# dfm/emcee

Measured on AMD Instinct MI355X. Metric: walker-updates/sec (whole node), 64-dim correlated Gaussian, StretchMove a=2, higher is better.
Workload: dtype f64

## Files before the change

emcee_amd/csrc/emx_kernels.hpp:

```cpp
#pragma once
#include <hip/hip_runtime.h>

#include <cstdint>
#include <type_traits>

#include "emx_planlog.hpp"
#include "emx_rng.hpp"

#ifndef EMX_OPT_RED4
#define EMX_OPT_RED4 1
#endif
#ifndef EMX_OPT_RTILE
#define EMX_OPT_RTILE 1
#endif
#ifndef EMX_LEAN_FOLD_D
#define EMX_LEAN_FOLD_D 0
#endif
#ifndef EMX_LEAN_FOLD_SPW
#define EMX_LEAN_FOLD_SPW 1
#endif
#ifndef EMX_OPT_SKEW
#define EMX_OPT_SKEW 1
#endif
#ifndef EMX_SNOOKER_BUDGET
#define EMX_SNOOKER_BUDGET 48
#endif
#ifndef EMX_STAMP_WAVE
#define EMX_STAMP_WAVE 0
#endif
#ifndef EMX_OPT_STAMPS
#define EMX_OPT_STAMPS 0
#endif
#ifndef EMX_EXPERIMENTS
#define EMX_EXPERIMENTS 0
#endif

namespace emx {

enum : int { MOVE_STRETCH = 0, MOVE_DE = 1, MOVE_SNOOKER = 2, MOVE_GAUSS = 3, MOVE_EVAL = 4,
             MOVE_WALK = 5, MOVE_KDE = 6,
             MOVE_MIX = 8  };
enum : int { GAUSS_VECTOR = 0, GAUSS_RANDOM = 1, GAUSS_SEQUENTIAL = 2 };
enum : int { TGT_NONE = 0, TGT_ISO = 1, TGT_DIAG = 2, TGT_DENSE = 3, TGT_ROSEN = 4, TGT_BOX = 5,
             TGT_REPLAY = 7, TGT_USER = 8 };
enum : uint32_t { ST_NAN_LOGP = 1u, ST_BAD_COORD = 2u, ST_EXCHANGE_OVERFLOW = 4u, ST_EXCHANGE_TIMEOUT = 8u,
                  ST_PLAN_PRODUCER = 16u,
                  ST_SINGULAR_COV = 32u };
constexpr int EMX_MAX_PEERS = 8;

__device__ __forceinline__ void raise_status(uint32_t* flags, uint32_t bit) {
    __hip_atomic_store(&flags[__builtin_ctz(bit)], 1u, __ATOMIC_RELAXED, __HIP_MEMORY_SCOPE_SYSTEM);
}

struct NativeArgs {
    uint64_t seed;
    uint64_t step;
    PermKey pk;
};

struct StepDesc {
    NativeArgs nat;
    long long stored_idx;
};
struct GraphCounters {
    unsigned long long step_base;
    long long stored_base;
};

struct HalfStepArgs {
    double* X;
    double* lp;
    uint8_t* acc;
    uint32_t* acc_count;
    double* chain;
    double* chain_lp;
    uint32_t* status;
    double* qout;
    double* fout;
    double* sendbuf;
    const int32_t* order;
    const int32_t* p0;
    const int32_t* p1;
    const int32_t* p2;
    const double* s0;
    const double* uacc;
    const double* logu;
    const double* fac;
    const double* tp0;
    const double* tp1;
    double tscale;
    double a;
    double sigma, g0;
    double gammas;
    int32_t N, D, S, split;
    int32_t pos0, ns;
    int32_t t_lo, t_hi;
    int32_t spw;
    int32_t target;
    int32_t Dp;
    int32_t ablate;
    const StepDesc* desc;
    double* chain_all;
    double* chain_lp_all;
    const int32_t* t_hi_dev;
    const double* disp;
    const double* gscale;
    double gsigma, gfac;
    unsigned long long gseed, gstep;
    unsigned long long* dbg;
    const struct PeerTable* peers;
    int32_t npeer;
    double* declp;
    const struct PeerTable* push_peers;
    long long push_off;
    int32_t npush;
    int32_t skew_sleep;
};

struct PeerTable {
    const double* X[EMX_MAX_PEERS];
    int32_t lo[EMX_MAX_PEERS];
};

template <int LEAN>
__device__ __forceinline__ const double* partner_base(const HalfStepArgs& A, int j) {
    if (LEAN == 1 || LEAN == 3 || LEAN == 4 || A.npeer == 0) return A.X;
    const PeerTable* __restrict__ T = A.peers;
    const double* b = T->X[0];
#pragma unroll
    for (int q = 1; q < EMX_MAX_PEERS; ++q) b = (q < A.npeer && j >= T->lo[q]) ? T->X[q] : b;
    return b;
}

template <int CTRL>
__device__ __forceinline__ double dpp_f64(double x) {
    const int lo = __builtin_amdgcn_update_dpp(0, __double2loint(x), CTRL, 0xf, 0xf, false);
    const int hi = __builtin_amdgcn_update_dpp(0, __double2hiint(x), CTRL, 0xf, 0xf, false);
    return __hiloint2double(hi, lo);
}

__device__ __forceinline__ double sum_swap16(double x) {
    const unsigned lo = (unsigned)__double2loint(x), hi = (unsigned)__double2hiint(x);
    const auto a = __builtin_amdgcn_permlane16_swap(lo, lo, false, false);
    const auto b = __builtin_amdgcn_permlane16_swap(hi, hi, false, false);
    return __hiloint2double((int)b[0], (int)a[0]) + __hiloint2double((int)b[1], (int)a[1]);
}

__device__ __forceinline__ double sum_swap32(double x) {
    const unsigned lo = (unsigned)__double2loint(x), hi = (unsigned)__double2hiint(x);
    const auto a = __builtin_amdgcn_permlane32_swap(lo, lo, false, false);
    const auto b = __builtin_amdgcn_permlane32_swap(hi, hi, false, false);
    return __hiloint2double((int)b[0], (int)a[0]) + __hiloint2double((int)b[1], (int)a[1]);
}

template <int G>
__device__ __forceinline__ double group_sum(double x) {
    if constexpr (G >= 2) x += dpp_f64<0xB1>(x);
    if constexpr (G >= 4) x += dpp_f64<0x4E>(x);
    if constexpr (G >= 8) x += dpp_f64<0x141>(x);
    if constexpr (G >= 16) x += dpp_f64<0x140>(x);
    if constexpr (G >= 32) x = sum_swap16(x);
    if constexpr (G >= 64) x = sum_swap32(x);
    return x;
}

__device__ __forceinline__ double row16_sum4(double v0, double v1, double v2, double v3, int lane) {
    const bool b0 = lane & 1, b1 = lane & 2;
    const double x = (b0 ? v1 : v0) + dpp_f64<0xB1>(b0 ? v0 : v1);
    const double y = (b0 ? v3 : v2) + dpp_f64<0xB1>(b0 ? v2 : v3);
    double z = (b1 ? y : x) + dpp_f64<0x4E>(b1 ? x : y);
    z += dpp_f64<0x124>(z);
    z += dpp_f64<0x128>(z);
    return z;
}

template <int G>
__device__ __forceinline__ bool group_any(bool pred, int sub) {
    const unsigned long long m = __ballot(pred);
    if constexpr (G == 64) {
        return m != 0ull;
    } else {
        return ((m >> (sub * G)) & ((1ull << G) - 1ull)) != 0ull;
    }
}
// ... 709 lines not shown
                    EMX_WAVE_SYNC();
                    double my_qf = 0.0;
                    {
                        const int am = lane & 15, ak = lane >> 4;
                        typedef double d4 __attribute__((ext_vector_type(4)));
                        double afr[KK];
#pragma unroll
                        for (int kk = 0; kk < KK; ++kk) {
                            if constexpr (RTILE)
                                afr[kk] = tile[am * RT + 4 * kk + ak];
                            else
                                afr[kk] = tile[am * RT + 4 * kk + ak] - muS[4 * kk + ak];
                        }
                        double part[4] = {0.0, 0.0, 0.0, 0.0};
                        if (EMX_OPT_STAMPS && A.dbg) { asm volatile("s_waitcnt lgkmcnt(0)" ::: "memory"); }
                        EMX_STAMP(5);
                        if (!(ablate_ & 1))
#pragma unroll
                        for (int nb = 0; nb < DPB; ++nb) {
                            d4 accv = {0.0, 0.0, 0.0, 0.0};
#pragma unroll
                            for (int kk = 4 * nb; kk < KK; ++kk)
                                accv = __builtin_amdgcn_mfma_f64_16x16x4f64(afr[kk], Sfrag[(dense_block(DPB, nb, kk >> 2) * 4 + (kk & 3)) * 64 + lane], accv, 0, 0, 0);
#pragma unroll
                            for (int r = 0; r < 4; ++r) part[r] = fma(accv[r], accv[r], part[r]);
                        }
                        if (EMX_OPT_STAMPS && A.dbg) { asm volatile("s_nop 0" ::: "memory"); }
                        EMX_STAMP(6);
#if EMX_OPT_RED4
                        my_qf = row16_sum4(part[0], part[1], part[2], part[3], lane);
#else
#pragma unroll
                        for (int r = 0; r < 4; ++r) part[r] = group_sum<16>(part[r]);
                        my_qf = part[0];
#pragma unroll
                        for (int r = 1; r < 4; ++r) my_qf = (am == r) ? part[r] : my_qf;
#endif
                    }
                    EMX_STAMP(7);
                    bool acc = false;
                    double lp_fin = my_lpo;
                    if (mine) {
                        const double lpn = -0.5 * my_qf;
                        if (lpn != lpn) raise_status(A.status, ST_NAN_LOGP);
                        if constexpr (MOVE == MOVE_EVAL) {
                            A.lp[my_i] = lpn;
                        } else {
                            const double lnpdiff = facS[myrow] + lpn - my_lpo;
                            acc = lnpdiff > my_logu;
                            A.acc[my_i] = acc ? 1 : 0;
                            if (acc) {
                                A.lp[my_i] = lpn;
                                lp_fin = lpn;
                            }
                            if (chain_lp_) {
                                chain_lp_[my_i] = lp_fin;
                                if (acc) A.acc_count[my_i] += 1u;
                            }
                            if (declp_) put_decision(t0 + tb + myrow - tlo_, acc ? lpn : __builtin_nan(""));
                        }
                    }
                    EMX_STAMP(8);
                    if constexpr (MOVE != MOVE_EVAL) {
                        const unsigned long long am64 = __ballot(acc);
                        if (sendbuf_ && (lane & 15) < 4) qfS[myrow] = lp_fin;
                        if (sendbuf_) EMX_WAVE_SYNC();
#pragma unroll
                        for (int pp = 0; pp < PPT; ++pp) {
                            if (ablate_ & 8) break;
                            const int row = pp * WPW + sub;
                            const int sidx = tb + row;
                            const bool lv = sidx < nslot;
                            const bool ac = lv && ((am64 >> ((row & 3) * 16 + (row >> 2))) & 1ull);
                            if (!lv) continue;
                            if (sendbuf_ && gl == 0) {
                                double* sb = sendbuf_ + (size_t)(t0 + sidx - tlo_) * (D + 2);
                                sb[D] = qfS[row];
                                sb[D + 1] = ac ? 1.0 : 0.0;
                            }
                            if (!ac) continue;
                            int wi2;
                            if constexpr (PF == PPT) {
                                wi2 = wi[0];
#pragma unroll
                                for (int k2 = 1; k2 < PF; ++k2) wi2 = (pp == k2) ? wi[k2] : wi2;
                            } else {
                                wi2 = A.order[pbase + sidx];
                            }
                            Row<G, V, CH> rr;
                            if constexpr (RTILE) {
                                rr = qk[pp < PF ? pp : 0];
                            } else {
#pragma unroll
                                for (int c = 0; c < CH; ++c)
#pragma unroll
                                    for (int v = 0; v < V; ++v) {
                                        const int d = (c * G + gl) * V + v;
                                        rr.x[c][v] = d < D ? tile[row * RT + d] : 0.0;
                                    }
                            }
                            store_row<G, V, CH>(rr, A.X + (size_t)wi2 * D, D, gl);
                            if (chain_) store_row_stream<G, V, CH>(rr, chain_ + (size_t)wi2 * D, D, gl);
                            if (sendbuf_) store_row<G, V, CH>(rr, sendbuf_ + (size_t)(t0 + sidx - tlo_) * (D + 2), D, gl);
                        }
                    }
                    EMX_STAMP(9);
                    EMX_WAVE_SYNC();
                }
            }
        }
    }
    if (EMX_OPT_STAMPS && A.dbg) { asm volatile("s_waitcnt vmcnt(0)" ::: "memory"); }
    EMX_STAMP(10);
    if (EMX_OPT_STAMPS && A.dbg && wib == 0 && lane == 0) A.dbg[(size_t)blockIdx.x * 16 + 12] = wall_clock64();
}

typedef unsigned int emx_u4 __attribute__((ext_vector_type(4)));
constexpr int EMX_CPOL_SC1 = 16;
template <int G, int V, int CH, int CPOL = EMX_CPOL_SC1>
__device__ __forceinline__ void load_row_agent(Row<G, V, CH>& r, __amdgpu_buffer_rsrc_t rsrc, int row, int D, int gl) {
    static_assert(V == 2 || V == 1, "two coordinates per lane and chunk (even ndim), or one (odd ndim: rows are 8-byte aligned only)");
    const int base = row * D;
    if constexpr (V == 1) {
        typedef unsigned int emx_u2 __attribute__((ext_vector_type(2)));
#pragma unroll
        for (int c = 0; c < CH; ++c) {
            const int d = c * G + gl;
            if (d < D) {
                const emx_u2 w = __builtin_amdgcn_raw_buffer_load_b64(rsrc, (base + d) * 8, 0, CPOL);
                double t;
                __builtin_memcpy(&t, &w, 8);
                r.x[c][0] = t;
            } else {
                r.x[c][0] = 0.0;
            }
        }
        return;
    }
#pragma unroll
    for (int c = 0; c < CH; ++c) {
        const int d = (c * G + gl) * V;
        if (d + 1 < D) {
            const emx_u4 w = __builtin_amdgcn_raw_buffer_load_b128(rsrc, (base + d) * 8, 0, CPOL);
            double2 t;
            __builtin_memcpy(&t, &w, 16);
            r.x[c][0] = t.x;
            r.x[c][1] = t.y;
        } else {
            r.x[c][0] = 0.0;
            r.x[c][1] = 0.0;
        }
    }
}
template <int G, int V, int CH, int CPOL = EMX_CPOL_SC1>
__device__ __forceinline__ void store_row_agent(const Row<G, V, CH>& r, __amdgpu_buffer_rsrc_t rsrc, int row, int D, int gl) {
    static_assert(V == 2 || V == 1, "two coordinates per lane and chunk (even ndim), or one (odd ndim)");
    const int base = row * D;
    if constexpr (V == 1) {
        typedef unsigned int emx_u2 __attribute__((ext_vector_type(2)));
#pragma unroll
        for (int c = 0; c < CH; ++c) {
            const int d = c * G + gl;
            if (d < D) {
                emx_u2 w;
                const double t = r.x[c][0];
                __builtin_memcpy(&w, &t, 8);
                __builtin_amdgcn_raw_buffer_store_b64(w, rsrc, (base + d) * 8, 0, CPOL);
            }
        }
        return;
    }
#pragma unroll
    for (int c = 0; c < CH; ++c) {
        const int d = (c * G + gl) * V;
        if (d + 1 < D) {
            const double2 t = {r.x[c][0], r.x[c][1]};
            emx_u4 w;
            __builtin_memcpy(&w, &t, 16);
            __builtin_amdgcn_raw_buffer_store_b128(w, rsrc, (base + d) * 8, 0, CPOL);
        }
    }
}
template <typename T>
__device__ __forceinline__ void store_agent(T* p, T v) { __hip_atomic_store(p, v, __ATOMIC_RELAXED, __HIP_MEMORY_SCOPE_AGENT); }
__device__ __forceinline__ double load_agent(const double* p) { return __hip_atomic_load(p, __ATOMIC_RELAXED, __HIP_MEMORY_SCOPE_AGENT); }
__device__ __forceinline__ unsigned load_agent(const unsigned* p) { return __hip_atomic_load(p, __ATOMIC_RELAXED, __HIP_MEMORY_SCOPE_AGENT); }
template <bool LOCAL, typename T>
__device__ __forceinline__ void store_scope(T* p, T v) {
    if constexpr (LOCAL)
        *p = v;
    else
        store_agent(p, v);
}

constexpr int PERSIST_MAX_ITERS = 40;
constexpr int PERSIST_BAR_STRIDE = 32;
constexpr int PERSIST_BAR_WORDS = 12 * PERSIST_BAR_STRIDE;
struct PersistIter {
    const char* plan;
    double *chain, *chain_lp;
    int32_t pos0, split;
    double gammas;
    int32_t kind, shift;
};
struct PersistCols {
    const int32_t *order, *p0, *p1, *p2;
    const double *s0, *logu, *fac;
    double *chain, *chain_lp;
    int32_t pos0, split;
    double gammas;
    int32_t kind, shift;
    __host__ __device__ __forceinline__ PersistCols(const PersistIter& it, size_t N)
        : order(reinterpret_cast<const int32_t*>(it.plan)), p0(reinterpret_cast<const int32_t*>(it.plan) + N),
          p1(reinterpret_cast<const int32_t*>(it.plan + N * 24)), p2(reinterpret_cast<const int32_t*>(it.plan + N * 24) + N),
          s0(reinterpret_cast<const double*>(it.plan + N * 8)), logu(reinterpret_cast<const double*>(it.plan + N * 32)),
          fac(reinterpret_cast<const double*>(it.plan + N * 32) + N), chain(it.chain), chain_lp(it.chain_lp), pos0(it.pos0), split(it.split),
          gammas(it.gammas), kind(it.kind), shift(it.shift) {}
};
struct PersistArgs {
    HalfStepArgs base;
    PersistIter it[PERSIST_MAX_ITERS];
    unsigned* bar;
    unsigned* ver;
    unsigned epoch0;
    unsigned lepoch0;
    unsigned hepoch0;
    unsigned long long timeout_ticks;
    int32_t niter;
    unsigned seq;
    unsigned* started_host;
    int32_t stagger;
};
static_assert(sizeof(PersistArgs) <= 4096, "kernel arguments of the persistent kernels");

__device__ __forceinline__ void persist_barrier_local(const PersistArgs& P, unsigned k, unsigned bid, unsigned ngroups) {
    asm volatile("s_waitcnt vmcnt(0)" ::: "memory");
    __syncthreads();
    if (threadIdx.x < 64) {
        const int lane = threadIdx.x;
        const __amdgpu_buffer_rsrc_t Fr = __builtin_amdgcn_make_buffer_rsrc((void*)(P.bar + 10 * PERSIST_BAR_STRIDE), 0, 64 * 4, 0x00020000);
        if (lane == 0) __builtin_amdgcn_raw_buffer_store_b32(k, Fr, (int)bid * 4, 0, 0);
        const unsigned long long t0 = wall_clock64();
        for (;;) {
            const unsigned v = __builtin_amdgcn_raw_buffer_load_b32(Fr, lane * 4, 0, EMX_CPOL_SC1);
            const bool ok = lane < (int)ngroups ? (int)(v - k) >= 0 : true;
            const bool dead = lane == 32 && v != 0u;
            if (__ballot(ok) == ~0ull || __ballot(dead) != 0ull) break;
            if (wall_clock64() - t0 > P.timeout_ticks) {
                if (lane == 0) {
                    raise_status(P.base.status, ST_EXCHANGE_TIMEOUT);
                    __hip_atomic_store(P.bar + 9 * PERSIST_BAR_STRIDE + 1, 2u, __ATOMIC_RELAXED, __HIP_MEMORY_SCOPE_AGENT);
                    __builtin_amdgcn_raw_buffer_store_b32(1u, Fr, 32 * 4, 0, 0);
                }
                break;
            }
        }
    }
    __syncthreads();
}

__device__ __forceinline__ void persist_barrier(const PersistArgs& P, unsigned k, unsigned long long* wall = nullptr) {
    asm volatile("s_waitcnt vmcnt(0)" ::: "memory");
    __syncthreads();
    if (threadIdx.x == 0) {
        const int xcd = blockIdx.x & 7;
        const unsigned per = (gridDim.x + 7 - xcd) / 8;
        unsigned* xctr = P.bar + xcd * PERSIST_BAR_STRIDE;
        unsigned* gctr = P.bar + 8 * PERSIST_BAR_STRIDE;
        unsigned* go = P.bar + 9 * PERSIST_BAR_STRIDE;
        if (wall) wall[0] = wall_clock64();
        const unsigned old = __hip_atomic_fetch_add(xctr, 1u, __ATOMIC_RELAXED, __HIP_MEMORY_SCOPE_AGENT);
        if (old == k * per - 1) {
            const unsigned o2 = __hip_atomic_fetch_add(gctr, 1u, __ATOMIC_RELAXED, __HIP_MEMORY_SCOPE_AGENT);
            if (o2 == k * 8 - 1) __hip_atomic_store(go, k, __ATOMIC_RELAXED, __HIP_MEMORY_SCOPE_AGENT);
        }
        const unsigned long long t0 = wall_clock64();
        for (;;) {
            const unsigned long long v = __hip_atomic_load(reinterpret_cast<unsigned long long*>(go), __ATOMIC_RELAXED, __HIP_MEMORY_SCOPE_AGENT);
            if ((int)((unsigned)v - k) >= 0 || (v >> 32) != 0ull) break;
            if (wall_clock64() - t0 > P.timeout_ticks) {
                raise_status(P.base.status, ST_EXCHANGE_TIMEOUT);
                __hip_atomic_store(go + 1, 2u, __ATOMIC_RELAXED, __HIP_MEMORY_SCOPE_AGENT);
                break;
            }
        }
        if (wall) wall[1] = wall_clock64();
    }
    __syncthreads();
}

__device__ __forceinline__ void persist_stagger_wait(int stagger, int wib) {
    const int how = stagger >> 8, cnt = stagger & 255;
    const int units = how == 0 ? (wib >> 2) : how == 1 ? (wib & 1) : how == 2 ? ((wib >> 1) & 1) : (wib & 3);
    for (int s = 0; s < cnt * units; ++s) __builtin_amdgcn_s_sleep(1);
}

template <bool LOCAL = false>
__device__ __forceinline__ bool persist_handshake(const PersistArgs& P) {
    __shared__ int ok_s;
    if (threadIdx.x == 0) {
        const unsigned k = LOCAL ? P.hepoch0 + 1u : P.epoch0 + 1u;
        const int xcd = LOCAL ? 0 : (int)(blockIdx.x & 7);
        const unsigned per = LOCAL ? gridDim.x >> 3 : (gridDim.x + 7 - xcd) / 8;
        unsigned* xctr = P.bar + xcd * PERSIST_BAR_STRIDE;
        unsigned* gctr = P.bar + 8 * PERSIST_BAR_STRIDE;
        unsigned* go = P.bar + 9 * PERSIST_BAR_STRIDE;
        int ok = 1;
        const unsigned long long v0 = __hip_atomic_load(reinterpret_cast<unsigned long long*>(go), __ATOMIC_RELAXED, __HIP_MEMORY_SCOPE_AGENT);
        if ((v0 >> 32) != 0ull) {
            ok = 0;
        } else {
            unsigned xcc = 0;
            if constexpr (LOCAL) {
                asm volatile("s_getreg_b32 %0, hwreg(HW_REG_XCC_ID)" : "=s"(xcc));
                __hip_atomic_fetch_or(go + 2, 1u << (xcc & 15u), __ATOMIC_RELAXED, __HIP_MEMORY_SCOPE_AGENT);
                asm volatile("s_waitcnt vmcnt(0)" ::: "memory");
            }
            const unsigned old = __hip_atomic_fetch_add(xctr, 1u, __ATOMIC_RELAXED, __HIP_MEMORY_SCOPE_AGENT);
            if (old == k * per - 1) {
                bool open = true;
                unsigned o2 = k * 8 - 1;
                if constexpr (LOCAL) {
                    const unsigned m = __hip_atomic_load(go + 2, __ATOMIC_RELAXED, __HIP_MEMORY_SCOPE_AGENT);
                    open = (m & (m - 1u)) == 0u;
                    if (open) {
                        __hip_atomic_store(go + 2, 0u, __ATOMIC_RELAXED, __HIP_MEMORY_SCOPE_AGENT);
                    } else {
                        raise_status(P.base.status, ST_EXCHANGE_TIMEOUT);
                        __hip_atomic_store(go + 1, 1u, __ATOMIC_RELAXED, __HIP_MEMORY_SCOPE_AGENT);
                    }
                } else {
                    o2 = __hip_atomic_fetch_add(gctr, 1u, __ATOMIC_RELAXED, __HIP_MEMORY_SCOPE_AGENT);
                }
                if (open && o2 == k * 8 - 1) {
                    __hip_atomic_store(go + 4, LOCAL ? (xcc & 15u) + 1u : 0u, __ATOMIC_RELAXED, __HIP_MEMORY_SCOPE_AGENT);
                    __hip_atomic_store(go + 3, P.seq, __ATOMIC_RELAXED, __HIP_MEMORY_SCOPE_AGENT);
                    if (P.started_host) __hip_atomic_store(P.started_host, P.seq, __ATOMIC_RELAXED, __HIP_MEMORY_SCOPE_SYSTEM);
                    __hip_atomic_store(go, k, __ATOMIC_RELAXED, __HIP_MEMORY_SCOPE_AGENT);
                }
            }
            const unsigned long long t0 = wall_clock64();
            for (;;) {
                const unsigned long long v = __hip_atomic_load(reinterpret_cast<unsigned long long*>(go), __ATOMIC_RELAXED, __HIP_MEMORY_SCOPE_AGENT);
                if ((v >> 32) != 0ull) {
                    ok = 0;
                    break;
                }
                if ((int)((unsigned)v - k) >= 0) break;
                if (wall_clock64() - t0 > P.timeout_ticks) {
                    raise_status(P.base.status, ST_EXCHANGE_TIMEOUT);
                    __hip_atomic_store(go + 1, 1u, __ATOMIC_RELAXED, __HIP_MEMORY_SCOPE_AGENT);
                    ok = 0;
                    break;
                }
            }
        }
        ok_s = ok;
    }
    __syncthreads();
    return ok_s != 0;
}

template <int G, int V, int CH, int DPB, int MOVE = MOVE_STRETCH, bool LOCAL = false, bool ROWS_LATE = false>
static __global__ __launch_bounds__(512) void k_persist(const PersistArgs P) {
    static_assert(MOVE == MOVE_STRETCH || MOVE == MOVE_DE || MOVE == MOVE_SNOOKER, "the red / blue moves");
    if (LOCAL && (blockIdx.x & 7u) != 0u) return;
    const unsigned bid = LOCAL ? blockIdx.x >> 3 : blockIdx.x, ngroups = LOCAL ? gridDim.x >> 3 : gridDim.x;
    constexpr int CPOL = EMX_CPOL_SC1;
    constexpr int CPOL_ST = LOCAL ? 0 : EMX_CPOL_SC1;
    constexpr bool DE = MOVE == MOVE_DE || MOVE == MOVE_SNOOKER;
    constexpr bool SN = MOVE == MOVE_SNOOKER;
    constexpr bool DEFER = !DE;
    constexpr int WPW = 64 / G;
    constexpr int PPT = 16 / WPW;
    constexpr int PF = PPT;
    static_assert(EMX_OPT_RTILE && EMX_OPT_RED4, "the persistent kernel is the one-tile-per-batch form");
    constexpr int Dp = DPB * 16, KK = Dp / 4, RT = Dp + 2;
    static_assert(G * V * CH >= Dp, "row layout must cover the padded dimension");
    extern __shared__ __attribute__((aligned(16))) double smem[];
    const HalfStepArgs& A = P.base;
    const int lane = threadIdx.x & 63;
    const int wib = threadIdx.x >> 6;
    const int sub = lane / G;
    const int gl = lane % G;
    const int D = A.D;
    double* Sfrag = smem;
    double* muS = smem + dense_img_doubles(Dp);
    double* tile = muS + Dp + (size_t)wib * (16 * RT + 32);
    double* qfS = tile + 16 * RT;
    double* facS = qfS + 16;
    {
        constexpr int IMG2 = (dense_img_doubles(Dp) + Dp) / 2;
        const double2* img = reinterpret_cast<const double2*>(A.tp1);
        double2* dst = reinterpret_cast<double2*>(smem);
        for (int e = threadIdx.x; e < IMG2; e += blockDim.x) dst[e] = img[e];
    }
    Row<G, V, CH> mu;
    load_row<G, V, CH>(mu, A.tp0, D, gl);
    if (!persist_handshake<LOCAL>(P)) return;
    const int wave = (int)bid * (blockDim.x >> 6) + wib;
    const int t0 = wave * 16;
    unsigned long long pst[6] = {0, 0, 0, 0, 0, 0}, pt = 0;
    const bool prof = EMX_OPT_STAMPS && A.dbg && wib == EMX_STAMP_WAVE;
    if (prof) {
        pt = __builtin_readcyclecounter();
        if (lane == 0) A.dbg[(size_t)bid * 16 + 11] = wall_clock64();
    }
#define EMX_PSTAMP(k_)                                                   \
    do {                                                                 \
        if (prof) {                                                      \
            const unsigned long long t_ = __builtin_readcyclecounter(); \
            pst[k_] += t_ - pt;                                          \
            pt = t_;                                                     \
        }                                                                \
    } while (0)
    const __amdgpu_buffer_rsrc_t Xr = __builtin_amdgcn_make_buffer_rsrc((void*)A.X, 0, A.N * D * 8, 0x00020000);
    const int myrow = (lane >> 4) + 4 * (lane & 3);
    const bool mine = (lane & 15) < 4;

    int wi[PF], ja[PF], jb[DE ? PF : 1], jc[SN ? PF : 1], my_i;
    double s0v[PF], facv[PF], my_logu, my_lpo;
    Row<G, V, CH> xi[PF];
    {
        const PersistCols I(P.it[0], (size_t)P.base.N);
        const int pbase = I.pos0 + t0;
#pragma unroll
        for (int k = 0; k < PF; ++k) {
            const int pos = pbase + k * WPW + sub;
            wi[k] = I.order[pos];
            ja[k] = I.p0[pos];
            if constexpr (DE) jb[k] = I.p1[pos];
            if constexpr (SN) jc[k] = I.p2[pos];
            s0v[k] = SN ? 0.0 : I.s0[pos];
            facv[k] = I.fac[pos];
        }
        my_i = I.order[pbase + myrow];
        my_logu = I.logu[pbase + myrow];
#pragma unroll
        for (int k = 0; k < PF; ++k) load_row_agent<G, V, CH, CPOL>(xi[k], Xr, wi[k], D, gl);
        my_lpo = load_agent(A.lp + my_i);
    }
    Row<G, V, CH> crow[DEFER ? PF : 1];
    int cwi[PF], cmy_i = 0;
    double clp = 0.0;
    double *cchain = nullptr, *cchain_lp = nullptr;
#pragma unroll
    for (int k = 0; k < PF; ++k) {
        if (DEFER || k == 0) crow[DEFER ? k : 0] = xi[k];
        cwi[k] = 0;
    }
    for (int n = 0; n < P.niter; ++n) {
        const PersistCols I(P.it[n], (size_t)P.base.N);
        Row<G, V, CH> xa[PF], xb[DE ? PF : 1], xc[SN ? PF : 1];
        persist_stagger_wait(P.stagger, wib);
#pragma unroll
        for (int k = 0; k < PF; ++k) {
            load_row_agent<G, V, CH, CPOL>(xa[k], Xr, ja[k], D, gl);
            if constexpr (DE) load_row_agent<G, V, CH, CPOL>(xb[k], Xr, jb[k], D, gl);
            if constexpr (SN) load_row_agent<G, V, CH, CPOL>(xc[k], Xr, jc[k], D, gl);
        }
        const bool more = n + 1 < P.niter;
        const PersistCols J(P.it[more ? n + 1 : n], (size_t)P.base.N);
        const bool pre = more && J.split != 0;
        const unsigned stamp = P.epoch0 + (unsigned)n + 1u;
        int wi_n[PF], ja_n[PF], jb_n[DE ? PF : 1], jc_n[SN ? PF : 1], my_i_n;
        double s0_n[PF], fac_n[PF], my_logu_n;
        {
            const int pbase = J.pos0 + t0;
#pragma unroll
            for (int k = 0; k < PF; ++k) {
                const int pos = pbase + k * WPW + sub;
                wi_n[k] = J.order[pos];
                ja_n[k] = J.p0[pos];
                if constexpr (DE) jb_n[k] = J.p1[pos];
                if constexpr (SN) jc_n[k] = J.p2[pos];
                s0_n[k] = SN ? 0.0 : J.s0[pos];
                fac_n[k] = J.fac[pos];
            }
            my_i_n = J.order[pbase + myrow];
            my_logu_n = J.logu[pbase + myrow];
        }
        if (prof) { asm volatile("s_waitcnt vmcnt(0)" ::: "memory"); }
        EMX_PSTAMP(0);
        Row<G, V, CH> qk[PF];
#pragma unroll
        for (int k = 0; k < PF; ++k) {
            const int srow = k * WPW + sub;
            double factor = facv[k];
            Row<G, V, CH> q;
            make_proposal<G, V, CH, MOVE>(xi[k], xa[k], xb[DE ? k : 0], xc[SN ? k : 0], s0v[k], A.gammas, D, gl, q, factor, ja[k]);
            bool bl = false;
#pragma unroll
            for (int c = 0; c < CH; ++c)
#pragma unroll
                for (int v = 0; v < V; ++v) bl |= !(fabs(q.x[c][v]) <= 1.79769313486231570815e308);
            const bool badq = group_any<G>(bl, sub);
            if (badq && gl == 0) raise_status(A.status, ST_BAD_COORD);
            const int trow = srow & 15;
#pragma unroll
            for (int c = 0; c < CH; ++c)
#pragma unroll
                for (int v = 0; v < V; ++v) {
                    const int d = (c * G + gl) * V + v;
                    if (d < Dp) tile[trow * RT + d] = !badq ? q.x[c][v] - mu.x[c][v] : 0.0;
                }
            qk[k] = q;
            if (gl == 0) facS[trow] = badq ? -__builtin_inf() : factor;
        }
        if (DEFER && cchain) {
#pragma unroll
            for (int k = 0; k < PF; ++k) store_row_stream<G, V, CH>(crow[k], cchain + (size_t)cwi[k] * D, D, gl);
            if (mine) cchain_lp[cmy_i] = clp;
            cchain = nullptr;
        }
        if (I.chain) {
#pragma unroll
            for (int k = 0; k < PF; ++k) {
                if constexpr (DEFER)
                    crow[k] = xi[k];
                else
                    store_row_stream<G, V, CH>(xi[k], I.chain + (size_t)wi[k] * D, D, gl);
            }
        }
        double my_lpo_n = 0.0;
        if (!ROWS_LATE && more) {
#pragma unroll
            for (int k = 0; k < PF; ++k) load_row_agent<G, V, CH, CPOL>(xi[k], Xr, wi_n[k], D, gl);
            my_lpo_n = load_agent(A.lp + my_i_n);
        }
        EMX_WAVE_SYNC();
        EMX_PSTAMP(1);
        double my_qf;
        {
            const int am = lane & 15, ak = lane >> 4;
            typedef double d4 __attribute__((ext_vector_type(4)));
            double afr[KK];
#pragma unroll
            for (int kk = 0; kk < KK; ++kk) afr[kk] = tile[am * RT + 4 * kk + ak];
            double part[4] = {0.0, 0.0, 0.0, 0.0};
#pragma unroll
            for (int nb = 0; nb < DPB; ++nb) {
                d4 accv = {0.0, 0.0, 0.0, 0.0};
#pragma unroll
                for (int kk = 4 * nb; kk < KK; ++kk)
                    accv = __builtin_amdgcn_mfma_f64_16x16x4f64(afr[kk], Sfrag[(dense_block(DPB, nb, kk >> 2) * 4 + (kk & 3)) * 64 + lane], accv, 0, 0, 0);
#pragma unroll
                for (int r = 0; r < 4; ++r) part[r] = fma(accv[r], accv[r], part[r]);
            }
            my_qf = row16_sum4(part[0], part[1], part[2], part[3], lane);
        }
        if (ROWS_LATE && more) {
            __builtin_amdgcn_sched_barrier(0);
#pragma unroll
            for (int k = 0; k < PF; ++k) load_row_agent<G, V, CH, CPOL>(xi[k], Xr, wi_n[k], D, gl);
            my_lpo_n = load_agent(A.lp + my_i_n);
            __builtin_amdgcn_sched_barrier(0);
        }
        if (prof) { asm volatile("s_nop 0" ::: "memory"); }
        EMX_PSTAMP(2);
        bool acc = false;
        if (mine) {
            const double lpn = -0.5 * my_qf;
            if (lpn != lpn) raise_status(A.status, ST_NAN_LOGP);
            const double lnpdiff = facS[myrow] + lpn - my_lpo;
            acc = lnpdiff > my_logu;
            store_scope<LOCAL>(A.acc + my_i, (uint8_t)(acc ? 1 : 0));
            if (acc) {
                store_scope<LOCAL>(A.lp + my_i, lpn);
                store_scope<LOCAL>(P.ver + my_i, stamp);
            }
            if (I.chain_lp) {
                if constexpr (DEFER)
                    clp = acc ? lpn : my_lpo;
                else
                    I.chain_lp[my_i] = acc ? lpn : my_lpo;
                if (acc) store_scope<LOCAL>(A.acc_count + my_i, load_agent(A.acc_count + my_i) + 1u);
            }
        }
        const unsigned long long am64 = __ballot(acc);
#pragma unroll
        for (int pp = 0; pp < PPT; ++pp) {
            const int row = pp * WPW + sub;
            const bool ac = (am64 >> ((row & 3) * 16 + (row >> 2))) & 1ull;
            if (ac) {
                store_row_agent<G, V, CH, CPOL_ST>(qk[pp], Xr, wi[pp], D, gl);
                if (I.chain) {
                    if constexpr (DEFER)
                        crow[pp] = qk[pp];
                    else
                        store_row_stream<G, V, CH>(qk[pp], I.chain + (size_t)wi[pp] * D, D, gl);
                }
            }
        }
        if (DEFER && I.chain) {
            cchain = I.chain;
            cchain_lp = I.chain_lp;
            cmy_i = my_i;
#pragma unroll
            for (int k = 0; k < PF; ++k) cwi[k] = wi[k];
        }
        EMX_WAVE_SYNC();
        EMX_PSTAMP(3);
        if (prof) {
            asm volatile("s_waitcnt vmcnt(0)" ::: "memory");
            EMX_PSTAMP(4);
        }
        if (!more) break;
        if constexpr (LOCAL)
            persist_barrier_local(P, P.lepoch0 + (unsigned)n + 1u, bid, ngroups);
        else
            persist_barrier(P, P.epoch0 + (unsigned)n + 2u,
                            (EMX_OPT_STAMPS && A.dbg) ? A.dbg + 4096 + ((size_t)n * ngroups + bid) * 2 : nullptr);
        EMX_PSTAMP(5);
#pragma unroll
        for (int k = 0; k < PF; ++k) {
            wi[k] = wi_n[k];
            ja[k] = ja_n[k];
            if constexpr (DE) jb[k] = jb_n[k];
            if constexpr (SN) jc[k] = jc_n[k];
            s0v[k] = s0_n[k];
            facv[k] = fac_n[k];
        }
        my_i = my_i_n;
        my_logu = my_logu_n;
        my_lpo = my_lpo_n;
        if (!pre) {
            unsigned vk[PF];
#pragma unroll
            for (int k = 0; k < PF; ++k) vk[k] = load_agent(P.ver + wi[k]);
            const unsigned vm = load_agent(P.ver + my_i);
#pragma unroll
            for (int k = 0; k < PF; ++k)
                if (vk[k] == stamp) load_row_agent<G, V, CH, CPOL>(xi[k], Xr, wi[k], D, gl);
            if (vm == stamp) my_lpo = load_agent(A.lp + my_i);
        }
    }
    if (DEFER && cchain) {
#pragma unroll
        for (int k = 0; k < PF; ++k) store_row_stream<G, V, CH>(crow[k], cchain + (size_t)cwi[k] * D, D, gl);
        if (mine) cchain_lp[cmy_i] = clp;
    }
    if (prof && lane == 0) {
        unsigned long long* o = A.dbg + (size_t)bid * 16;
#pragma unroll
        for (int k = 0; k < 6; ++k) o[k] = pst[k];
        o[6] = (unsigned long long)P.niter;
        o[12] = wall_clock64();
    }
#undef EMX_PSTAMP
}

constexpr int SMALL_MAX_MOVES = 8;
struct GaussGen {
    unsigned long long gseed, gstep;
    double gfac, gsigma;
    const double* gscale;
};
constexpr int PERSIST_GAUSS_MAX_STEPS = 16;
struct PersistGaussStep {
    const int32_t* p0;
    const double* logu;
    double *chain, *chain_lp;
    unsigned long long gstep;
    double gfac;
};
struct PersistGaussArgs {
    HalfStepArgs base;
    PersistGaussStep st[PERSIST_GAUSS_MAX_STEPS];
    int32_t nsteps;
};

template <int G, int V, int CH, int DPB>
static __global__ __launch_bounds__(512) void k_persist_gauss(const PersistGaussArgs P) {
    constexpr int MOVE = MOVE_GAUSS;
    constexpr int WPW = 64 / G;
    constexpr int PPT = 16 / WPW;
    constexpr int Dp = DPB * 16, KK = Dp / 4, RT = Dp + 2;
    static_assert(EMX_OPT_RTILE && EMX_OPT_RED4 && G * V * CH >= Dp, "the one-tile-per-batch form");
    extern __shared__ __attribute__((aligned(16))) double smem[];
    const HalfStepArgs& A = P.base;
    const int lane = threadIdx.x & 63;
    const int wib = threadIdx.x >> 6;
    const int sub = lane / G;
    const int gl = lane % G;
    const int D = A.D;
    double* Sfrag = smem;
    double* muS = smem + dense_img_doubles(Dp);
    double* tile = muS + Dp + (size_t)wib * (16 * RT + 32);
    double* facS = tile + 16 * RT + 16;
    {
        constexpr int IMG2 = (dense_img_doubles(Dp) + Dp) / 2;
        const double2* img = reinterpret_cast<const double2*>(A.tp1);
        double2* dst = reinterpret_cast<double2*>(smem);
        for (int e = threadIdx.x; e < IMG2; e += blockDim.x) dst[e] = img[e];
    }
    Row<G, V, CH> mu;
    load_row<G, V, CH>(mu, A.tp0, D, gl);
    __syncthreads();
    const int wave = blockIdx.x * (blockDim.x >> 6) + wib;
    const int w0 = wave * 16;
    const int myrow = (lane >> 4) + 4 * (lane & 3);
    const bool mine = (lane & 15) < 4;
    const int my_i = w0 + myrow;
    Row<G, V, CH> xi[PPT];
#pragma unroll
    for (int k = 0; k < PPT; ++k) load_row<G, V, CH>(xi[k], A.X + (size_t)(w0 + k * WPW + sub) * D, D, gl);
    double my_lp = A.lp[my_i];
    bool my_acc = false;
    for (int s = 0; s < P.nsteps; ++s) {
        const PersistGaussStep& S = P.st[s];
        GaussGen gg;
        gg.gseed = A.gseed;
        gg.gstep = S.gstep;
        gg.gfac = S.gfac;
        gg.gsigma = A.gsigma;
        gg.gscale = A.gscale;
        const double my_logu = S.logu[my_i];
        Row<G, V, CH> qk[PPT];
#pragma unroll
        for (int k = 0; k < PPT; ++k) {
            const int i = w0 + k * WPW + sub;
            const int col = S.p0[i];
            Row<G, V, CH> xa, q;
            gauss_disp_row<G, V, CH>(xa, gg, i, col, D, gl);
            double factor = 0.0;
            make_proposal<G, V, CH, MOVE>(xi[k], xa, xa, xa, 0.0, A.gammas, D, gl, q, factor, col);
            bool bl = false;
#pragma unroll
            for (int c = 0; c < CH; ++c)
#pragma unroll
                for (int v = 0; v < V; ++v) bl |= !(fabs(q.x[c][v]) <= 1.79769313486231570815e308);
            const bool badq = group_any<G>(bl, sub);
            if (badq && gl == 0) raise_status(A.status, ST_BAD_COORD);
            const int trow = (k * WPW + sub) & 15;
#pragma unroll
            for (int c = 0; c < CH; ++c)
#pragma unroll
                for (int v = 0; v < V; ++v) {
                    const int d = (c * G + gl) * V + v;
                    if (d < Dp) tile[trow * RT + d] = !badq ? q.x[c][v] - mu.x[c][v] : 0.0;
                }
            qk[k] = q;
            if (gl == 0) facS[trow] = badq ? -__builtin_inf() : factor;
        }
        EMX_WAVE_SYNC();
        double my_qf;
        {
            const int am = lane & 15, ak = lane >> 4;
            typedef double d4 __attribute__((ext_vector_type(4)));
            double afr[KK];
#pragma unroll
            for (int kk = 0; kk < KK; ++kk) afr[kk] = tile[am * RT + 4 * kk + ak];
            double part[4] = {0.0, 0.0, 0.0, 0.0};
#pragma unroll
            for (int nb = 0; nb < DPB; ++nb) {
                d4 accv = {0.0, 0.0, 0.0, 0.0};
#pragma unroll
                for (int kk = 4 * nb; kk < KK; ++kk)
                    accv = __builtin_amdgcn_mfma_f64_16x16x4f64(afr[kk], Sfrag[(dense_block(DPB, nb, kk >> 2) * 4 + (kk & 3)) * 64 + lane], accv, 0, 0, 0);
#pragma unroll
                for (int r = 0; r < 4; ++r) part[r] = fma(accv[r], accv[r], part[r]);
            }
            my_qf = row16_sum4(part[0], part[1], part[2], part[3], lane);
        }
        bool acc = false;
        if (mine) {
            const double lpn = -0.5 * my_qf;
            if (lpn != lpn) raise_status(A.status, ST_NAN_LOGP);
            const double lnpdiff = facS[myrow] + lpn - my_lp;
            acc = lnpdiff > my_logu;
            if (acc) my_lp = lpn;
            my_acc = acc;
            if (S.chain_lp) {
                S.chain_lp[my_i] = my_lp;
                if (acc) A.acc_count[my_i] += 1u;
            }
        }
        const unsigned long long am64 = __ballot(acc);
#pragma unroll
        for (int pp = 0; pp < PPT; ++pp) {
            const int row = pp * WPW + sub;
            const bool ac = (am64 >> ((row & 3) * 16 + (row >> 2))) & 1ull;
            if (ac) xi[pp] = qk[pp];
            if (S.chain) store_row_stream<G, V, CH>(xi[pp], S.chain + (size_t)(w0 + row) * D, D, gl);
        }
        EMX_WAVE_SYNC();
    }
#pragma unroll
    for (int k = 0; k < PPT; ++k) store_row<G, V, CH>(xi[k], A.X + (size_t)(w0 + k * WPW + sub) * D, D, gl);
    if (mine) {
        A.lp[my_i] = my_lp;
        A.acc[my_i] = my_acc ? 1 : 0;
    }
}

constexpr int SMALL_ANY_MOVE = 7;

__host__ __device__ inline int native_move_choice(uint64_t seed, uint64_t step, const double* cdf, int n) {
    const Philox4 r = philox4x32_10((uint32_t)step, (uint32_t)(step >> 32), 0x4d4f5645u , 0, (uint32_t)seed,
                                    (uint32_t)(seed >> 32));
// ... 1390 lines not shown
```

Before: 3.381 billion.

## Issue next-iteration partner row loads right after the grid barrier

Partner-row loads (xa/xb/xc) are hoisted out of the loop top and issued immediately after the persistent barrier, before the version checks and conditional reloads of own rows. Their latency then overlaps the stale-row reload path. A new branch-free flat loader sends out-of-range lanes to an out-of-bounds offset so the buffer load returns zeros, and it skips chunks beyond the padded dimension. It also adds profiling counters split by iteration kind, which cost extra registers only when stamps are enabled.

```diff
diff --git a/emcee_amd/csrc/emx_kernels.hpp b/emcee_amd/csrc/emx_kernels.hpp
--- a/emcee_amd/csrc/emx_kernels.hpp
+++ b/emcee_amd/csrc/emx_kernels.hpp
@@ -30,6 +30,9 @@
 #endif
 #ifndef EMX_OPT_STAMPS
 #define EMX_OPT_STAMPS 0
+#endif
+#ifndef EMX_OPT_BOUNDARY
+#define EMX_OPT_BOUNDARY 1
 #endif
 #ifndef EMX_EXPERIMENTS
 #define EMX_EXPERIMENTS 0
@@ -1045,6 +1048,32 @@
         }
     }
 }
+template <int G, int V, int CH, int NC, int CPOL = EMX_CPOL_SC1>
+__device__ __forceinline__ void load_row_agent_flat(Row<G, V, CH>& r, __amdgpu_buffer_rsrc_t rsrc, int row, int D, int gl, int oob) {
+    static_assert(V == 2 || V == 1, "two coordinates per lane and chunk (even ndim), or one (odd ndim)");
+    static_assert(NC <= CH, "chunks of the row");
+    const int base = row * D;
+#pragma unroll
+    for (int c = 0; c < CH; ++c) {
+        const int d = (c * G + gl) * V;
+        if (c >= NC) {
+#pragma unroll
+            for (int v = 0; v < V; ++v) r.x[c][v] = 0.0;
+        } else if constexpr (V == 1) {
+            typedef unsigned int emx_u2 __attribute__((ext_vector_type(2)));
+            const emx_u2 w = __builtin_amdgcn_raw_buffer_load_b64(rsrc, d < D ? (base + d) * 8 : oob, 0, CPOL);
+            double t;
+            __builtin_memcpy(&t, &w, 8);
+            r.x[c][0] = t;
+        } else {
+            const emx_u4 w = __builtin_amdgcn_raw_buffer_load_b128(rsrc, d + 1 < D ? (base + d) * 8 : oob, 0, CPOL);
+            double2 t;
+            __builtin_memcpy(&t, &w, 16);
+            r.x[c][0] = t.x;
+            r.x[c][1] = t.y;
+        }
+    }
+}
 template <int G, int V, int CH, int CPOL = EMX_CPOL_SC1>
 __device__ __forceinline__ void store_row_agent(const Row<G, V, CH>& r, __amdgpu_buffer_rsrc_t rsrc, int row, int D, int gl) {
     static_assert(V == 2 || V == 1, "two coordinates per lane and chunk (even ndim), or one (odd ndim)");
@@ -1267,6 +1296,7 @@
     constexpr int WPW = 64 / G;
     constexpr int PPT = 16 / WPW;
     constexpr int PF = PPT;
+    constexpr bool BOUNDARY = EMX_OPT_BOUNDARY != 0;
     static_assert(EMX_OPT_RTILE && EMX_OPT_RED4, "the persistent kernel is the one-tile-per-batch form");
     constexpr int Dp = DPB * 16, KK = Dp / 4, RT = Dp + 2;
     static_assert(G * V * CH >= Dp, "row layout must cover the padded dimension");
@@ -1294,6 +1324,8 @@
     const int wave = (int)bid * (blockDim.x >> 6) + wib;
     const int t0 = wave * 16;
     unsigned long long pst[6] = {0, 0, 0, 0, 0, 0}, pt = 0;
+    unsigned long long pstk[2][6] = {{0, 0, 0, 0, 0, 0}, {0, 0, 0, 0, 0, 0}}, pcnt[2] = {0, 0}, pbar[2] = {0, 0};
+    int pkind = -1;
     const bool prof = EMX_OPT_STAMPS && A.dbg && wib == EMX_STAMP_WAVE;
     if (prof) {
         pt = __builtin_readcyclecounter();
@@ -1304,6 +1336,8 @@
         if (prof) {                                                      \
             const unsigned long long t_ = __builtin_readcyclecounter(); \
             pst[k_] += t_ - pt;                                          \
+            if (pkind == 0) pstk[0][k_] += t_ - pt;                      \
+            if (pkind == 1) pstk[1][k_] += t_ - pt;                      \
             pt = t_;                                                     \
         }                                                                \
     } while (0)
@@ -1342,16 +1376,29 @@
         if (DEFER || k == 0) crow[DEFER ? k : 0] = xi[k];
         cwi[k] = 0;
     }
+    Row<G, V, CH> xa[PF], xb[DE ? PF : 1], xc[SN ? PF : 1];
+    constexpr int NCH = (Dp + G * V - 1) / (G * V) < CH ? (Dp + G * V - 1) / (G * V) : CH;
+    const int xoob = A.N * D * 8;
+    auto partner_rows = [&]() {
+        persist_stagger_wait(P.stagger, wib);
+#pragma unroll
+        for (int k = 0; k < PF; ++k) {
+            if constexpr (BOUNDARY) {
+                load_row_agent_flat<G, V, CH, NCH, CPOL>(xa[k], Xr, ja[k], D, gl, xoob);
+                if constexpr (DE) load_row_agent_flat<G, V, CH, NCH, CPOL>(xb[k], Xr, jb[k], D, gl, xoob);
+                if constexpr (SN) load_row_agent_flat<G, V, CH, NCH, CPOL>(xc[k], Xr, jc[k], D, gl, xoob);
+            } else {
+                load_row_agent<G, V, CH, CPOL>(xa[k], Xr, ja[k], D, gl);
+                if constexpr (DE) load_row_agent<G, V, CH, CPOL>(xb[k], Xr, jb[k], D, gl);
+                if constexpr (SN) load_row_agent<G, V, CH, CPOL>(xc[k], Xr, jc[k], D, gl);
+            }
+        }
+    };
+    if (BOUNDARY && P.niter > 0) partner_rows();
     for (int n = 0; n < P.niter; ++n) {
         const PersistCols I(P.it[n], (size_t)P.base.N);
-        Row<G, V, CH> xa[PF], xb[DE ? PF : 1], xc[SN ? PF : 1];
-        persist_stagger_wait(P.stagger, wib);
-#pragma unroll
-        for (int k = 0; k < PF; ++k) {
-            load_row_agent<G, V, CH, CPOL>(xa[k], Xr, ja[k], D, gl);
-            if constexpr (DE) load_row_agent<G, V, CH, CPOL>(xb[k], Xr, jb[k], D, gl);
-            if constexpr (SN) load_row_agent<G, V, CH, CPOL>(xc[k], Xr, jc[k], D, gl);
-        }
+        if (prof && pkind >= 0) pcnt[pkind] += 1;
+        if constexpr (!BOUNDARY) partner_rows();
         const bool more = n + 1 < P.niter;
         const PersistCols J(P.it[more ? n + 1 : n], (size_t)P.base.N);
         const bool pre = more && J.split != 0;
@@ -1505,6 +1552,11 @@
             persist_barrier(P, P.epoch0 + (unsigned)n + 2u,
                             (EMX_OPT_STAMPS && A.dbg) ? A.dbg + 4096 + ((size_t)n * ngroups + bid) * 2 : nullptr);
         EMX_PSTAMP(5);
+        if (prof) {
+            if (pkind >= 0) pbar[pkind] += 1;
+            pkind = pre ? 0 : 1;
+        }
+        if constexpr (BOUNDARY) __builtin_amdgcn_s_waitcnt(0x0F70);
 #pragma unroll
         for (int k = 0; k < PF; ++k) {
             wi[k] = wi_n[k];
@@ -1517,15 +1569,35 @@
         my_i = my_i_n;
         my_logu = my_logu_n;
         my_lpo = my_lpo_n;
+        unsigned vk[PF], vm = 0u;
         if (!pre) {
-            unsigned vk[PF];
 #pragma unroll
             for (int k = 0; k < PF; ++k) vk[k] = load_agent(P.ver + wi[k]);
-            const unsigned vm = load_agent(P.ver + my_i);
-#pragma unroll
-            for (int k = 0; k < PF; ++k)
-                if (vk[k] == stamp) load_row_agent<G, V, CH, CPOL>(xi[k], Xr, wi[k], D, gl);
-            if (vm == stamp) my_lpo = load_agent(A.lp + my_i);
+            vm = load_agent(P.ver + my_i);
+            if constexpr (!BOUNDARY) {
+#pragma unroll
+                for (int k = 0; k < PF; ++k)
+                    if (vk[k] == stamp) load_row_agent<G, V, CH, CPOL>(xi[k], Xr, wi[k], D, gl);
+                if (vm == stamp) my_lpo = load_agent(A.lp + my_i);
+            }
+        }
+        if constexpr (BOUNDARY) {
+            partner_rows();
+            if (!pre) {
+                __builtin_amdgcn_sched_barrier(0);
+                unsigned mk[PF], mm = vm == stamp ? 1u : 0u;
+#pragma unroll
+                for (int k = 0; k < PF; ++k) {
+                    mk[k] = vk[k] == stamp ? 1u : 0u;
+                    asm volatile("" : "+v"(mk[k]));
+                }
+                asm volatile("" : "+v"(mm));
+                __builtin_amdgcn_sched_barrier(0);
+#pragma unroll
+                for (int k = 0; k < PF; ++k)
+                    if (mk[k]) load_row_agent<G, V, CH, CPOL>(xi[k], Xr, wi[k], D, gl);
+                if (mm) my_lpo = load_agent(A.lp + my_i);
+            }
         }
     }
     if (DEFER && cchain) {
@@ -1539,6 +1611,18 @@
         for (int k = 0; k < 6; ++k) o[k] = pst[k];
         o[6] = (unsigned long long)P.niter;
         o[12] = wall_clock64();
+        if (bid < 2048u) {
+            unsigned long long* ok = A.dbg + 32768 + (size_t)bid * 16;
+#pragma unroll
+            for (int k = 0; k < 6; ++k) {
+                ok[k] = pstk[0][k];
+                ok[6 + k] = pstk[1][k];
+            }
+            ok[12] = pcnt[0];
+            ok[13] = pcnt[1];
+            ok[14] = pbar[0];
+            ok[15] = pbar[1];
+        }
     }
 #undef EMX_PSTAMP
 }
```

Result: no change. 3.386 billion (median of 3 runs) (+0.1%).
